# Wikinaut/agrep

Measured on NVIDIA H100. Metric: text_scan_throughput, higher is better.
Workload: dtype u32 bitwise

## Files before the change

### agrep_b200/csrc/refine.cu

```cuda
#include "scan_internal.cuh"


#define REFINE_MAXG  8
int refine_launch_u32a(int nrows, const RefineParams &P, unsigned &grid, cudaStream_t st);
int refine_launch_u32b(int nrows, const RefineParams &P, unsigned &grid, cudaStream_t st);
int refine_launch_u64(int nrows, const RefineParams &P, unsigned &grid, cudaStream_t st);
int refine_launch_costs(bool narrow, int nrows, const RefineParams &P, unsigned &grid, cudaStream_t st);

__global__ void __launch_bounds__(REFINE_THREADS)
k_compact_ranges(const uint32_t *bitmap, uint64_t n_words, const uint64_t *range_offsets, uint64_t *list, uint64_t cap)
{
	const uint32_t lane = threadIdx.x & 31;
	const uint64_t warp = ((uint64_t)blockIdx.x * REFINE_THREADS + threadIdx.x) >> 5, nwarps = ((uint64_t)gridDim.x * REFINE_THREADS) >> 5;
	const uint64_t n_groups = (n_words + 31) / 32, per = (n_groups + nwarps - 1) / nwarps;
	const uint64_t g_begin = warp * per < n_groups ? warp * per : n_groups, g_end = (g_begin + per < n_groups) ? g_begin + per : n_groups;
	uint64_t at = range_offsets[warp];
	for (uint64_t g0 = g_begin; g0 < g_end; g0 += 8) {
		uint32_t wd[8];
#pragma unroll
		for (int u = 0; u < 8; u++) { const uint64_t w = (g0 + u) * 32 + lane; wd[u] = (g0 + u < g_end && w < n_words) ? bitmap[w] : 0u; }
#pragma unroll
		for (int u = 0; u < 8; u++) {
			const uint32_t word = wd[u];
			if (!__ballot_sync(0xffffffffu, word != 0)) continue;
			const uint64_t w = (g0 + u) * 32 + lane;
			uint32_t c = __popc(word), pre = c;
#pragma unroll
			for (int o = 1; o < 32; o <<= 1) { uint32_t v = __shfl_up_sync(0xffffffffu, pre, o); if (lane >= (uint32_t)o) pre += v; }
			const uint32_t total = __shfl_sync(0xffffffffu, pre, 31);
			uint64_t mine = at + (pre - c);
			for (uint32_t b = word; b; b &= b - 1) { if (mine < cap) list[mine] = w * 32 + (uint64_t)(__ffs(b) - 1); mine++; }
			at += total;
		}
	}
}

static bool refine_geometry(const agb_desc &d, RefineParams &P)
{
	if (!front_usable(d) || !d.refine) return false;
	int max_off = 0, min_off = 1 << 30;
	for (int i = 0; i < d.n_anchors; i++) { max_off = std::max(max_off, (int)d.anchor_off[i]); min_off = std::min(min_off, (int)d.anchor_off[i]); }
	for (int i = 0; i < d.n_anchors3; i++) { max_off = std::max(max_off, (int)d.anchor3_off[i]); min_off = std::min(min_off, (int)d.anchor3_off[i]); }
	P.lo_off = max_off + d.k;
	P.hi_off = 15 + d.pat_len - min_off + d.k;
	P.gb = (P.lo_off + 15) / 16;
	P.ng = P.gb + (P.hi_off + 15) / 16;
	if (P.ng < P.gb + 2) P.ng = P.gb + 2;
	const int pw = (d.pat_len + 3) / 4, ngc = (d.engine != AGB_ENGINE_ASEARCH1 && d.M <= 31 && pw <= 4) ? 4 : REFINE_MAXG;
	if (!(P.ng <= ngc && max_off <= 31 && d.pat_len >= 1 && d.pat_len <= 64)) return false;
	const int na = d.n_anchors + d.n_anchors3;
	if (na > 16) return false;
	uint32_t val[16], msk[16]; int off[16];
	for (int i = 0; i < d.n_anchors; i++) { val[i] = d.anchor[i]; msk[i] = d.anchor_mask; off[i] = d.anchor_off[i]; }
	for (int i = 0; i < d.n_anchors3; i++) { val[d.n_anchors + i] = d.anchor3[i]; msk[d.n_anchors + i] = 0x00FFFFFFu; off[d.n_anchors + i] = d.anchor3_off[i]; }
	for (int i = 0; i < na; i++) for (int j = 0; j < i; j++) if ((val[i] & msk[j]) == val[j] || (val[j] & msk[i]) == val[i]) return false;
	uint32_t mul = 0x9E3779B1u;
	for (int attempt = 0; attempt < 4096; attempt++, mul = mul * 0x2C1B3C6Du + 0x297A2D39u) {
		int8_t slot[32]; bool ok = true;
		memset(slot, 0, sizeof slot);
		mul |= 1u;
		for (int i = 0; i < na && ok; i++) {
			const uint32_t h = (val[i] * mul) >> 27;
			if (slot[h]) ok = false; else slot[h] = (int8_t)(i + 1);
		}
		if (!ok) continue;
// ... 5 lines not shown
		return true;
	}
	return false;
}

static void refine_t1_setup(const agb_desc &d, RefineParams &P)
{
	uint8_t lit[64]; bool is_lit[64]; bool fold = false; int n_lit = 0;
	for (int j = 0; j < d.pat_len; j++) {
		const uint64_t bit = 1ull << (d.M - (d.L + 2 + j));
		int cnt = 0, c0 = -1, c1 = -1;
		for (int c = 0; c < 256; c++) if (d.mask[c] & bit) { if (cnt == 0) c0 = c; else if (cnt == 1) c1 = c; cnt++; }
		is_lit[j] = false; lit[j] = 0;
		if (cnt == 1 && c0 < 0x80) { is_lit[j] = true; lit[j] = (uint8_t)c0; }
		else if (cnt == 2 && (c0 ^ c1) == 0x20 && c1 < 0x80) { is_lit[j] = true; lit[j] = (uint8_t)(c0 | 0x20); fold = true; }
		if (is_lit[j]) n_lit++;
	}
	P.t1 = 0;
	if (n_lit <= d.k + 1) return;
	P.t1 = 1; P.t1_fold = fold ? 0x20202020u : 0u;
	for (int w = 0; w < 16; w++) { P.t1_pat[w] = 0; P.t1_care[w] = 0; }
	for (int j = 0; j < d.pat_len; j++) if (is_lit[j]) {
		P.t1_pat[j >> 2] |= (uint32_t)(fold ? (lit[j] | 0x20) : lit[j]) << (8 * (j & 3));
		P.t1_care[j >> 2] |= 0x80u << (8 * (j & 3));
	}
}

int refine_launch(const agb_desc &d, Workspace &W, const void *d_text, uint64_t n, cudaStream_t st, bool *ran)
{
	RefineParams P; memset(&P, 0, sizeof P);
	*ran = false;
	if (n == 0 || !refine_geometry(d, P)) return AGB_OK;
	const uint64_t n_chunks = (n + 15) / 16, n_words = (n_chunks + 31) / 32;
	P.text = (const uint8_t *)d_text; P.bitmap = W.bitmap; P.out = W.bitmap2; P.warp_counts = W.range_counts;
	P.n = n; P.n_chunks = n_chunks; P.n_words = n_words; P.desc = W.d_desc;
	P.fold = d.anchor_fold; P.amask = d.anchor_mask; P.na = d.n_anchors; P.k = d.k; P.pat_len = d.pat_len;
	for (int i = 0; i < d.n_anchors; i++) { P.anchor[i] = d.anchor[i]; P.off[i] = d.anchor_off[i]; }
	{
		bool distinct = true;
		for (int i = 0; i < d.n_anchors; i++) for (int j = 0; j < i; j++) if (d.anchor[i] == d.anchor[j]) distinct = false;
		P.one = 1; P.scale = 1;
		for (int i = d.anchor_len; i < 4; i++) P.scale <<= 8;
		P.poly = (distinct && poly_setup(d.anchor, d.n_anchors, 8 * d.anchor_len, P.coef)) ? 1 : 0;
		P.n3 = 0;
		if (d.n_anchors3) {
			uint32_t c3[AGB_MAXANCHOR];
			if (!P.poly || !poly_setup(d.anchor3, d.n_anchors3, 24, c3)) return AGB_OK;
			P.n3 = d.n_anchors3;
			for (int i = 0; i < d.n_anchors3; i++) P.coef3[i] = c3[i];
		}
	}
	refine_t1_setup(d, P);
	unsigned grid = refine_grid(W, n);
	P.sm_count = W.sm_count;
	const bool costs = d.engine == AGB_ENGINE_ASEARCH1, narrow = d.M <= 31;
	int rc = costs ? refine_launch_costs(narrow, d.nrows, P, grid, st)
	       : !narrow ? refine_launch_u64(d.nrows, P, grid, st)
	       : d.nrows <= 4 ? refine_launch_u32a(d.nrows, P, grid, st) : refine_launch_u32b(d.nrows, P, grid, st);
	if (rc) return AGB_ERR_ARG;
	g_launches++;
	CUDA_TRY(cudaGetLastError());
	W.refine_ctas = grid;
	*ran = true;
	return AGB_OK;
}

unsigned refine_grid(const Workspace &W, uint64_t n)
{
	const uint64_t n_chunks = (n + 15) / 16, n_words = (n_chunks + 31) / 32, groups = (n_words + 31) / 32;
	unsigned grid = (unsigned)std::min<uint64_t>((groups + 3) / 4, (uint64_t)W.sm_count * 16);
	return grid ? grid : 1;
}

int compact_ranges_launch(Workspace &W, uint64_t n, cudaStream_t st)
{
	const uint64_t n_chunks = (n + 15) / 16, n_words = (n_chunks + 31) / 32;
	const unsigned grid = W.refine_ctas;
	k_compact_ranges<<<grid, REFINE_THREADS, 0, st>>>(W.bitmap2, n_words, W.range_offsets, W.cand, W.cand_cap); g_launches++;
	CUDA_TRY(cudaGetLastError());
	return AGB_OK;
}
```

### agrep_b200/csrc/refine_kernel.cuh

```cuda
#ifndef AGB_REFINE_KERNEL_CUH
#define AGB_REFINE_KERNEL_CUH
#include "automaton.cuh"

#define REFINE_RING1 544
#define REFINE_RING2 64
#define REFINE_RING3 128
#define REFINE_MAXG  8
#define REFINE_PAD   32

struct AnchorTable { int8_t idx[32]; uint32_t val[16], mask[16]; int8_t off[16]; int n; };
__device__ __forceinline__ uint32_t hit_windows_tab(const uint32_t (&x)[5], const AnchorTable &A)
{
	uint32_t hits = 0;
#pragma unroll
	for (int w = 0; w < 4; w++) {
		const uint32_t wv[4] = { x[w], __funnelshift_r(x[w], x[w + 1], 8), __funnelshift_r(x[w], x[w + 1], 16), __funnelshift_r(x[w], x[w + 1], 24) };
		for (int a = 0; a < A.n; a++) {
			const uint32_t V = A.val[a], M = A.mask[a];
#pragma unroll
			for (int j = 0; j < 4; j++) if ((wv[j] & M) == V) hits |= 1u << (4 * w + j);
		}
	}
	return hits;
}
// ... 93 lines not shown
		for (int i = 0; i < NWT; i++) W[i] = __funnelshift_r(W[i], W[i + 1], 8);
	}
	int miss = 0;
#pragma unroll
	for (int w = 0; w < NW; w++) miss += __popc(acc[w] & P.t1_care[w]);
	return miss <= P.k;
}

template <typename T, int NR, bool COSTS>
__device__ __forceinline__ bool window_passes(const uint8_t *bytes, const bool run, const int wlen, const T init0,
                                              const T *mask, const DevConsts<T> &C)
{
	T S[NR];
#pragma unroll
	for (int r = 0; r < NR; r++) S[r] = init0;
	int q = 0;
	for (; q + 4 <= wlen; q += 4) {
		int c[4];
#pragma unroll
		for (int i = 0; i < 4; i++) c[i] = run ? (int)__ldg(bytes + q + i) : 0;
		T m[4];
#pragma unroll
		for (int i = 0; i < 4; i++) m[i] = mask[c[i]];
#pragma unroll
		for (int i = 0; i < 4; i++) rows_step<T, NR, COSTS>(S, m[i], C);
	}
	for (; q < wlen; q++) {
		const int c = run ? (int)__ldg(bytes + q) : 0;
		rows_step<T, NR, COSTS>(S, mask[c], C);
	}
	return run && (S[NR - 1] & C.endpos) != 0;
}

struct Refill { uint32_t word, next_word; uint32_t half; };
__device__ __forceinline__ void refine_refill(const RefineParams &P, Refill &R, uint32_t *ring, uint32_t &count, uint32_t lane,
                                              uint64_t &g, uint64_t g_begin, uint64_t g_end)
{
	if (R.half == 0) {
		const uint64_t w = g * 32 + lane;
		R.word = R.next_word;
		if (w < P.n_words) P.out[w] = 0u;
		R.next_word = (g + 1 < g_end && w + 32 < P.n_words) ? P.bitmap[w + 32] : 0u;
	}
	const uint32_t word = ((lane >> 4) == R.half) ? R.word : 0u;
	uint32_t c = __popc(word), pre = c;
#pragma unroll
	for (int o = 1; o < 32; o <<= 1) { uint32_t v = __shfl_up_sync(0xffffffffu, pre, o); if (lane >= (uint32_t)o) pre += v; }
	const uint32_t total = __shfl_sync(0xffffffffu, pre, 31);
	pre += count - c;
	const uint32_t rel0 = (uint32_t)(g - g_begin) * 1024u + lane * 32u;
	for (uint32_t b = word; b; b &= b - 1) ring[pre++] = rel0 + (uint32_t)(__ffs(b) - 1);
	count += total;
	if (R.half) g++;
	R.half ^= 1u;
	__syncwarp();
}

template <typename T, int NR, bool COSTS, int NW>
__global__ void __launch_bounds__(REFINE_THREADS, 6)
k_refine(const RefineParams P)
{
	constexpr int NGC = NW <= 4 ? 4 : REFINE_MAXG;
	constexpr int NWT = NW + (2 * (NR - 1) + 3) / 4;
	extern __shared__ __align__(16) uint32_t s_strip[];
	__shared__ RecShared<T, NR> SH;
	__shared__ uint32_t s_ring1[REFINE_THREADS / 32][REFINE_RING1];
	__shared__ uint32_t s_ring2[REFINE_THREADS / 32][REFINE_RING2];
	__shared__ uint32_t s_ring3[REFINE_THREADS / 32][REFINE_RING3];
	__shared__ AnchorTable s_offs;
	if (threadIdx.x == 0) {
#pragma unroll
		for (int i = 0; i < 32; i++) s_offs.idx[i] = (int8_t)(P.hidx64[i >> 3] >> (8 * (i & 7)));
#pragma unroll
		s_offs.n = P.na + P.n3;
#pragma unroll
		for (int i = 0; i < 16; i++) { s_offs.val[i] = P.hval[i]; s_offs.mask[i] = P.hmask[i]; s_offs.off[i] = (int8_t)(P.hoffs64[i >> 3] >> (8 * (i & 7))); }
	}
	DevConsts<T> C;
	shared_init<T, NR>(SH, C, P.desc, REFINE_THREADS);
	const T init0 = mirror<T>((T)P.desc->init0);
	const int wlen = P.pat_len + 2 * P.k;
	const uint32_t lane = threadIdx.x & 31, wib = threadIdx.x >> 5, lt_mask = (1u << lane) - 1u;
	uint32_t *ring1 = s_ring1[wib], *ring2 = s_ring2[wib], *ring3 = s_ring3[wib];
	const int stride_w = P.ng * 4 + 1;
	uint32_t *strip = s_strip + threadIdx.x * stride_w;
	const uint32_t *cw = strip + P.gb * 4;
	const int so0 = P.gb * 16 - 32 - P.k;

	const uint64_t warp = ((uint64_t)blockIdx.x * REFINE_THREADS + threadIdx.x) >> 5, nwarps = ((uint64_t)gridDim.x * REFINE_THREADS) >> 5;
	const uint64_t n_groups = (P.n_words + 31) / 32, per = (n_groups + nwarps - 1) / nwarps;
	const uint64_t g_begin = warp * per < n_groups ? warp * per : n_groups, g_end = (g_begin + per < n_groups) ? g_begin + per : n_groups;
	const uint64_t chunk0 = g_begin * 1024;
	uint32_t rel_lo, rel_hi;
	{
		const int64_t lo_chunk = ((int64_t)P.lo_off + 15) / 16;
		int64_t hi_chunk = ((int64_t)P.n - P.hi_off - 16) / 16;
		if ((int64_t)P.n - P.hi_off - 16 < 0) hi_chunk = -1;
		if (hi_chunk > (int64_t)P.n_chunks - 3) hi_chunk = (int64_t)P.n_chunks - 3;
		const int64_t a = lo_chunk - (int64_t)chunk0, b = hi_chunk - (int64_t)chunk0;
		rel_lo = a < 0 ? 0u : (a > 0x7fffffff ? 0x7fffffffu : (uint32_t)a);
		rel_hi = b < 0 ? 0u : (b > 0x7fffffff ? 0x7fffffffu : (uint32_t)b);
		if (b < 0) rel_lo = 0x7fffffffu;
	}
	const uint4 *text4 = reinterpret_cast<const uint4 *>(P.text) + chunk0;
	uint32_t kept = 0;
	auto keep_chunk = [&](uint32_t rel) {
		const uint64_t chunk = chunk0 + rel;
		const uint32_t bit = 1u << (chunk & 31);
		const uint32_t old = atomicOr(&P.out[chunk >> 5], bit);
		kept += (old & bit) ? 0u : 1u;
	};

	uint32_t n1 = 0, n2 = 0, n3 = 0;
	uint64_t g = g_begin;
	Refill RF; RF.word = 0; RF.half = 0;
	RF.next_word = (g < g_end && g * 32 + lane < P.n_words) ? P.bitmap[g * 32 + lane] : 0u;
	auto fill1 = [&]() { while (n1 < 32 && g < g_end) refine_refill(P, RF, ring1, n1, lane, g, g_begin, g_end); };
	uint32_t nrel = 0; bool nrun = false, nedge = false; uint4 nx[NGC];
	auto pop_load = [&](uint32_t rel, bool active) {
		nrel = rel;
		nedge = active && (rel < rel_lo || rel > rel_hi);
		nrun = active && !nedge;
		if (nrun) {
			const uint4 *src = text4 + ((int64_t)rel - P.gb);
#pragma unroll
			for (int gi = 0; gi < NGC; gi++) if (gi < P.ng) nx[gi] = __ldg(src + gi);
		}
	};
	auto to_strip = [&]() {
#pragma unroll
		for (int gi = 0; gi < NGC; gi++) if (gi < P.ng) {
			strip[gi * 4 + 0] = nx[gi].x; strip[gi * 4 + 1] = nx[gi].y; strip[gi * 4 + 2] = nx[gi].z; strip[gi * 4 + 3] = nx[gi].w;
		}
	};
	auto count_push = [&](uint32_t rel, uint32_t code, bool run) {
		const bool pass = run && (!P.t1 || band_count_passes<NW, NWT, COSTS ? 0 : 2 * (NR - 1) + 1>(P, strip, so0 + (int)code));
		const uint32_t pm = __ballot_sync(0xffffffffu, pass);
		if (pass) ring3[n3 + __popc(pm & lt_mask)] = (rel << 6) | code;
		n3 += __popc(pm);
	};
	auto walk_batch = [&]() {
		const uint32_t m = n3 < 32 ? n3 : 32;
		const bool run = lane < m;
		const uint32_t e = run ? ring3[n3 - m + lane] : 0u;
		n3 -= m;
		const uint8_t *wbytes = P.text + ((int64_t)(chunk0 + (e >> 6)) * 16 + (int64_t)(e & 63u) - 32 - P.k);
		if (window_passes<T, NR, COSTS>(run ? wbytes : P.text, run, wlen, init0, SH.mask, C)) keep_chunk(e >> 6);
		__syncwarp();
	};
	auto more_batch = [&]() {
		const uint32_t m = n2 < 32 ? n2 : 32;
		const bool run = lane < m;
		const uint32_t e = run ? ring2[n2 - m + lane] : 0u;
		n2 -= m;
		const uint32_t rel = e >> 6, first = e & 63u;
		if (run) {
			const uint4 *src = text4 + ((int64_t)rel - P.gb);
#pragma unroll
			for (int gi = 0; gi < NGC; gi++) if (gi < P.ng) {
				const uint4 v = __ldg(src + gi);
				strip[gi * 4 + 0] = v.x; strip[gi * 4 + 1] = v.y; strip[gi * 4 + 2] = v.z; strip[gi * 4 + 3] = v.w;
			}
		}
		uint32_t hits = 0;
		if (run) {
			const uint32_t x[5] = { cw[0] | P.fold, cw[1] | P.fold, cw[2] | P.fold, cw[3] | P.fold, cw[4] | P.fold };
			hits = P.n3 ? hit_windows_tab(x, s_offs) : hit_windows(x, P);
			hits &= hits - 1;
		}
		uint32_t seen1 = first, seen2 = first;
		for (int it = 0; it < 3; it++) {
			if (!__ballot_sync(0xffffffffu, hits != 0)) break;
			uint32_t code = first; bool fresh = false;
			if (hits) {
				code = start_code(cw, __ffs(hits) - 1, P, s_offs);
				hits &= hits - 1;
				fresh = code != first && code != seen1 && code != seen2;
				seen2 = seen1; seen1 = code;
			}
			count_push(rel, code, fresh);
		}
		if (hits) keep_chunk(rel);
		__syncwarp();
	};
	auto pop1 = [&]() {
		const uint32_t m = n1 < 32 ? n1 : 32;
		const bool active = lane < m;
		pop_load(active ? ring1[n1 - m + lane] : 0u, active);
		n1 -= m;
	};

	bool have = false;
	for (;;) {
		if (n3 >= 32) { walk_batch(); continue; }
		if (n2 >= 32) { more_batch(); continue; }
		if (!have) {
			fill1();
			if (n1 == 0) break;
			pop1(); have = true;
			continue;
		}
		const uint32_t crel = nrel; const bool crun = nrun, cedge = nedge;
		if (crun) to_strip();
		fill1();
		have = n1 != 0;
		if (have) pop1();
		if (cedge) keep_chunk(crel);
		uint32_t hits = 0, code = 0;
		if (crun) {
			const uint32_t x[5] = { cw[0] | P.fold, cw[1] | P.fold, cw[2] | P.fold, cw[3] | P.fold, cw[4] | P.fold };
			hits = P.n3 ? hit_windows_tab(x, s_offs) : hit_windows(x, P);
			if (hits) code = start_code(cw, __ffs(hits) - 1, P, s_offs);
		}
		count_push(crel, code, hits != 0);
		{
			uint32_t rest = hits & (hits - 1);
			if (rest && !(rest & (rest - 1)) && start_code(cw, __ffs(rest) - 1, P, s_offs) == code) rest = 0;
			const bool more = rest != 0;
			const uint32_t mm = __ballot_sync(0xffffffffu, more);
			if (more) ring2[n2 + __popc(mm & lt_mask)] = (crel << 6) | code;
			n2 += __popc(mm);
		}
		__syncwarp();
	}
	while (n2 || n3) { if (n3 >= 32 || !n2) walk_batch(); else more_batch(); }
	const uint32_t total = __reduce_add_sync(0xffffffffu, kept);
	if (lane == 0) P.warp_counts[warp] = total;
}

template <typename T, int NR, bool COSTS, int NW>
static void launch_refine_nw(const RefineParams &P, unsigned &grid, cudaStream_t st)
{
	const size_t smem = ((size_t)REFINE_THREADS * (P.ng * 4 + 1) + REFINE_PAD) * sizeof(uint32_t);
	int per_sm = 0;
	if (cudaOccupancyMaxActiveBlocksPerMultiprocessor(&per_sm, k_refine<T, NR, COSTS, NW>, REFINE_THREADS, smem) != cudaSuccess || per_sm < 1) per_sm = 4;
	grid = std::min<unsigned>(grid, (unsigned)per_sm * (unsigned)P.sm_count);
	if (!grid) grid = 1;
	k_refine<T, NR, COSTS, NW><<<grid, REFINE_THREADS, smem, st>>>(P);
}
template <typename T, int NR, bool COSTS>
static void launch_refine_one(const RefineParams &P, unsigned &grid, cudaStream_t st)
{
	const int pw = (P.pat_len + 3) / 4;
	if (COSTS) { if (sizeof(T) == 4) launch_refine_nw<T, NR, COSTS, 8>(P, grid, st); else launch_refine_nw<T, NR, COSTS, 16>(P, grid, st); return; }
	if (sizeof(T) == 4) {
		if (pw <= 2) launch_refine_nw<T, NR, COSTS, 2>(P, grid, st);
		else if (pw == 3) launch_refine_nw<T, NR, COSTS, 3>(P, grid, st);
		else if (pw == 4) launch_refine_nw<T, NR, COSTS, 4>(P, grid, st);
		else if (pw <= 6) launch_refine_nw<T, NR, COSTS, 6>(P, grid, st);
		else launch_refine_nw<T, NR, COSTS, 8>(P, grid, st);
	} else {
		if (pw <= 8) launch_refine_nw<T, NR, COSTS, 8>(P, grid, st);
		else if (pw <= 12) launch_refine_nw<T, NR, COSTS, 12>(P, grid, st);
// ... 6 lines not shown
```

### agrep_b200/csrc/scan.cu

```cuda
#include "scan_internal.cuh"
#include "corpus.h"
#include <unistd.h>
#include <fcntl.h>
#include <sys/stat.h>
#include <functional>
#include <memory>
#include <mutex>
#include <thread>

thread_local char g_err[512];
std::atomic<uint64_t> g_launches{0};

extern "C" const char *agb_last_error(void) { return g_err; }
extern "C" const char *agb_version(void) { return "agrep-b200 0.1 (sm_90a)"; }
extern "C" uint64_t agb_kernel_launches(void) { return g_launches.load(); }
static void host_release(int dev);
extern "C" void agb_shutdown(void)
{
	int cur = 0; cudaGetDevice(&cur);
	for (int dev = 0; dev < 64; dev++) {
		host_release(dev);
		std::lock_guard<std::mutex> lk(g_ws_mu[dev]);
		Workspace &W = g_ws[dev];
		if (!W.totals && !W.bitmap) continue;
		if (cudaSetDevice(dev) != cudaSuccess) { cudaGetLastError(); continue; }
		cudaDeviceSynchronize();
		cudaFree(W.bitmap); cudaFree(W.bitmap2); cudaFree(W.range_counts); cudaFree(W.range_offsets);
		cudaFree(W.tile_counts); cudaFree(W.tile_offsets); cudaFree(W.cand); cudaFree(W.cand_counts); cudaFree(W.cand_offsets);
		cudaFree(W.cand_first); cudaFree(W.scan_sums); cudaFree(W.scan_offs); cudaFree(W.ord_blocks); cudaFree(W.totals);
		cudaFreeHost(W.h_totals); cudaFree(W.d_desc); cudaFree(W.d_gram); cudaFreeHost(W.h_gram);
		cudaFree(W.d_regex);
		if (W.e0) cudaEventDestroy(W.e0); if (W.e1) cudaEventDestroy(W.e1); if (W.e2) cudaEventDestroy(W.e2);
		W = Workspace();
	}
	cudaSetDevice(cur);
}
extern "C" int agb_device_count(void) { int n = 0; if (cudaGetDeviceCount(&n) != cudaSuccess) return 0; return n; }
extern "C" int agb_set_device(int dev) { CUDA_TRY(cudaSetDevice(dev)); return AGB_OK; }


Workspace g_ws[64];
std::mutex g_ws_mu[64];

static int ws_prepare(Workspace &W, uint64_t n)
{
	if (!W.totals) {
		CUDA_TRY(cudaMalloc(&W.totals, 24 * sizeof(unsigned long long)));
		CUDA_TRY(cudaMallocHost(&W.h_totals, 24 * sizeof(unsigned long long)));
		CUDA_TRY(cudaMalloc(&W.d_desc, sizeof(agb_desc)));
		CUDA_TRY(cudaMalloc(&W.range_counts, REFINE_MAX_RANGES * sizeof(uint32_t)));
		CUDA_TRY(cudaMalloc(&W.range_offsets, REFINE_MAX_RANGES * sizeof(uint64_t)));
		CUDA_TRY(cudaEventCreate(&W.e0)); CUDA_TRY(cudaEventCreate(&W.e1)); CUDA_TRY(cudaEventCreate(&W.e2));
		int dev = 0; CUDA_TRY(cudaGetDevice(&dev));
		CUDA_TRY(cudaDeviceGetAttribute(&W.sm_count, cudaDevAttrMultiProcessorCount, dev));
	}
	uint64_t n_chunks = (n + 15) / 16, n_words = (n_chunks + 31) / 32, tiles = (n + std::min<uint64_t>(DENSE_TILE, SL_TILE) - 1) / std::min<uint64_t>(DENSE_TILE, SL_TILE) + 1;
	size_t bb = (size_t)(n_words + FRONT_WORDS_PER_STAGE) * 4;
	if (bb > W.bitmap_bytes) {
		if (W.bitmap) cudaFree(W.bitmap);
		if (W.bitmap2) cudaFree(W.bitmap2);
		W.bitmap = nullptr; W.bitmap2 = nullptr; W.bitmap_bytes = 0;
		CUDA_TRY(cudaMalloc(&W.bitmap, bb));
		CUDA_TRY(cudaMalloc(&W.bitmap2, bb)); W.bitmap_bytes = bb;
	}
	if (tiles + 1 > W.tiles) {
		if (W.tile_counts) cudaFree(W.tile_counts);
		if (W.tile_offsets) cudaFree(W.tile_offsets);
		W.tile_counts = nullptr; W.tile_offsets = nullptr; W.tiles = 0;
		CUDA_TRY(cudaMalloc(&W.tile_counts, (tiles + 1) * sizeof(uint32_t)));
		CUDA_TRY(cudaMalloc(&W.tile_offsets, (tiles + 1) * sizeof(uint64_t)));
		W.tiles = tiles + 1;
	}
	return AGB_OK;
}

static int ws_cand_reserve(Workspace &W, size_t want_cand)
{
	want_cand = std::max<size_t>(want_cand, (size_t)1 << 20);
	if (want_cand > W.cand_cap) {
		want_cand += want_cand / 4;
		if (W.cand) cudaFree(W.cand);
		if (W.cand_counts) cudaFree(W.cand_counts);
		if (W.cand_offsets) cudaFree(W.cand_offsets);
		if (W.cand_first) cudaFree(W.cand_first);
		if (W.scan_sums) cudaFree(W.scan_sums);
		if (W.scan_offs) cudaFree(W.scan_offs);
		W.cand = nullptr; W.cand_counts = nullptr; W.cand_offsets = nullptr; W.cand_first = nullptr; W.cand_cap = 0;
		W.scan_sums = nullptr; W.scan_offs = nullptr; W.scan_cap = 0;
		CUDA_TRY(cudaMalloc(&W.cand_first, want_cand * sizeof(agb_record)));
		W.scan_cap = want_cand / SCAN_BLOCK + 2;
		CUDA_TRY(cudaMalloc(&W.scan_sums, W.scan_cap * sizeof(uint32_t)));
		CUDA_TRY(cudaMalloc(&W.scan_offs, W.scan_cap * sizeof(uint64_t)));
		CUDA_TRY(cudaMalloc(&W.cand, want_cand * sizeof(uint64_t)));
		CUDA_TRY(cudaMalloc(&W.cand_counts, want_cand * sizeof(uint32_t)));
		CUDA_TRY(cudaMalloc(&W.cand_offsets, want_cand * sizeof(uint64_t)));
		W.cand_cap = want_cand;
// ... 22 lines not shown
		CUDA_TRY(cudaMemcpyAsync(W.d_regex, tab, bytes, cudaMemcpyHostToDevice, st));
		CUDA_TRY(cudaStreamSynchronize(st));
		memcpy(W.h_regex, tab, bytes); W.regex_bytes = bytes;
	}
	W.regex_tail = rx->tail;
	return AGB_OK;
}

static int list_stage(const agb_desc &d, Workspace &W, RecParams &P, bool want_list, cudaStream_t st)
{
	P.cand = W.cand; P.cand_cap = W.cand_cap; P.tile_counts = W.cand_counts; P.tile_offsets = W.cand_offsets;
	P.cand_first = want_list ? W.cand_first : nullptr;
	const unsigned grid = (unsigned)std::min<uint64_t>((W.cand_cap + REC_THREADS - 1) / REC_THREADS, (uint64_t)W.sm_count * 16);
	if (launch_records_list(d, P, grid, st)) return AGB_ERR_ARG;
	CUDA_TRY(cudaGetLastError());
	if (want_list) {
		const unsigned nb = (unsigned)((W.cand_cap + SCAN_BLOCK - 1) / SCAN_BLOCK);
		k_scan_partial<<<nb, 1024, 0, st>>>(W.cand_counts, W.cand_cap, W.scan_sums, W.totals + 12);
		k_scan_tiles<<<1, 1024, 0, st>>>(W.scan_sums, W.scan_offs, nb, nullptr);
		k_scan_apply<<<nb, 1024, 0, st>>>(W.cand_counts, W.cand_cap, W.scan_offs, W.cand_offsets, W.totals + 12);
		g_launches += 3;
		P.emit = 1;
		if (launch_records_list(d, P, grid, st)) return AGB_ERR_ARG;
		CUDA_TRY(cudaGetLastError());
	}
	return AGB_OK;
}

static int records_launch(const agb_desc &d, Workspace &W, const void *d_text, uint64_t n, bool use_front, bool refined, int want,
                          int want_level, agb_record *d_records, uint64_t capacity, cudaStream_t st, const ShardInfo *sh)
{
	const uint64_t n_chunks = (n + 15) / 16, n_words = (n_chunks + 31) / 32, tiles = (n_words + REC_THREADS - 1) / REC_THREADS;
	RecParams P; memset(&P, 0, sizeof P);
	P.text = (const uint8_t *)d_text; P.bitmap = use_front ? (refined ? W.bitmap2 : W.bitmap) : nullptr;
	P.n = n; P.n_chunks = n_chunks; P.n_words = n_words; P.desc = W.d_desc;
	P.records = d_records; P.capacity = capacity;
	P.totals = W.totals; P.emit = 0; P.levels = (want & AGB_WANT_LEVELS) ? 1 : 0; P.want_level = want_level;
	P.own_lo = sh ? sh->own_lo : INT64_MIN; P.own_hi = sh ? sh->own_hi : INT64_MAX; P.shard_last = sh ? sh->last : 1;
	P.rx_tab = W.d_regex; P.rx_tail = W.regex_tail;
	if (!tiles) return AGB_OK;
	const bool want_list = (want & AGB_WANT_RECORDS) && capacity;
	if (d.engine == AGB_ENGINE_REGEX) {
		P.tile_counts = W.tile_counts; P.tile_offsets = W.tile_offsets;
		const uint64_t rtiles = (n + DENSE_TILE - 1) / DENSE_TILE;
		if (launch_regex(d, P, (unsigned)rtiles, st)) return AGB_ERR_ARG;
		CUDA_TRY(cudaGetLastError());
		if (want_list) {
			k_scan_tiles<<<1, 1024, 0, st>>>(W.tile_counts, W.tile_offsets, rtiles, nullptr); g_launches++;
			P.emit = 1;
			if (launch_regex(d, P, (unsigned)rtiles, st)) return AGB_ERR_ARG;
			CUDA_TRY(cudaGetLastError());
		}
		return AGB_OK;
	}
	if (use_front && refined) {
		int rc = ws_cand_reserve(W, std::max<size_t>(W.cand_hint + W.cand_hint / 4, (size_t)(n_chunks / 512) + 65536)); if (rc) return rc;
		const unsigned ranges = W.refine_ctas * (REFINE_THREADS / 32);
		k_scan_tiles<<<1, 1024, 0, st>>>(W.range_counts, W.range_offsets, ranges, W.totals + 12); g_launches++;
		rc = compact_ranges_launch(W, n, st); if (rc) return rc;
		return list_stage(d, W, P, want_list, st);
	}
	if (use_front) {
		const uint64_t blocks = (n_words + COMPACT_THREADS * COMPACT_WPT - 1) / (COMPACT_THREADS * COMPACT_WPT);
		k_compact_count<<<(unsigned)blocks, COMPACT_THREADS, 0, st>>>(W.bitmap, n_words, W.tile_counts, W.totals); g_launches++;
		k_scan_tiles<<<1, 1024, 0, st>>>(W.tile_counts, W.tile_offsets, blocks, W.totals + 12); g_launches++;
		CUDA_TRY(cudaMemcpyAsync(W.h_totals + 12, W.totals + 12, sizeof(unsigned long long), cudaMemcpyDeviceToHost, st));
		CUDA_TRY(cudaStreamSynchronize(st));
// ... 844 lines not shown
```

### agrep_b200/csrc/scan_internal.cuh

```cuda
#ifndef AGB_SCAN_INTERNAL_CUH
#define AGB_SCAN_INTERNAL_CUH
#include "agrep_b200.h"
#include "pattern_internal.h"
#include <cuda_runtime.h>
#include <stdint.h>
#include <stdio.h>
#include <string.h>
#include <stdlib.h>
#include <atomic>
#include <algorithm>

extern thread_local char g_err[512];
extern std::atomic<uint64_t> g_launches;

#define CUDA_TRY(x) do { cudaError_t e_ = (x); if (e_ != cudaSuccess) { \
	snprintf(g_err, sizeof g_err, "%s failed: %s (%s:%d)", #x, cudaGetErrorString(e_), __FILE__, __LINE__); \
	return AGB_ERR_CUDA; } } while (0)

#define FRONT_THREADS 256
#define FRONT_CH      4
#define FRONT_STAGE_CHUNKS (FRONT_THREADS * FRONT_CH)
#define FRONT_STAGE_BYTES  (FRONT_STAGE_CHUNKS * 16)
#define FRONT_SLOT_BYTES   (FRONT_STAGE_BYTES + 16)
#define FRONT_NST     2
#define FRONT_CTAS_PER_SM 6
#define FRONT_WORDS_PER_STAGE (FRONT_STAGE_CHUNKS / 32)

struct FrontParams {
	const uint8_t *text;
	uint32_t    *bitmap;
	uint64_t     n;
	uint64_t     n_chunks;
	uint64_t     readable;
	uint64_t     stage_begin, stage_end;
	uint32_t     fold, amask;
	uint32_t     one, scale;
	uint32_t     anchor[AGB_MAXANCHOR];
	uint32_t     coef[AGB_MAXANCHOR];
	int          n3;
	uint32_t     s256;
	int          alen;
	uint32_t     coef3[4];
	uint16_t    *nl_blocks;
	uint32_t     delim4, dfold4;
};
#define FRONT_SMEM (FRONT_NST * FRONT_SLOT_BYTES)

#define REFINE_THREADS 128
struct RefineParams {
	const uint8_t *text; const uint32_t *bitmap; uint32_t *out; uint32_t *warp_counts;
	uint64_t n, n_chunks, n_words;
	const agb_desc *desc;
	uint32_t fold, amask; int na, k, pat_len;
	int gb, ng;
	int lo_off, hi_off;
	uint32_t anchor[AGB_MAXANCHOR]; int32_t off[AGB_MAXANCHOR];
	uint32_t coef[AGB_MAXANCHOR]; uint32_t one, scale; int poly;
	int t1, t1_words;
	uint32_t t1_fold, t1_pat[16], t1_care[16];
	uint32_t hmul; uint64_t hidx64[4];
	uint32_t hval[16], hmask[16]; uint64_t hoffs64[2];
	int n3; uint32_t coef3[4];
	int sm_count;
};

#define REC_THREADS 128

struct RecParams {
	const uint8_t  *text;
	const uint32_t *bitmap;
	uint64_t n, n_chunks, n_words;
	const agb_desc *desc;
	uint32_t *tile_counts;
	const uint64_t *tile_offsets;
	agb_record *records; uint64_t capacity;
	unsigned long long *totals;
	const uint64_t *cand; uint64_t cand_cap;
	agb_record *cand_first;
	int emit;
	int levels;
	int want_level;
	int warm;
	int64_t own_lo, own_hi; int shard_last;
// ... 10 lines not shown
#define SL_TILE    (SL_THREADS * SL_PER)
#define SL_APRON   128
#define SL_STRIDE  (SL_PER + 4)
#define SL_SMEM    ((SL_THREADS + 1) * SL_STRIDE + 12)
#define COMPACT_THREADS 256
#define COMPACT_WPT 4
#define SCAN_BLOCK 16384

#define ORD_THREADS 256
#define ORD_TILE    32768
#define ORD_PER     (ORD_TILE / ORD_THREADS)
#define ORD_BLOCK   512

struct OrdParams {
	const uint8_t *text; uint64_t n;
	uint16_t *blocks; uint32_t *tiles; const uint64_t *tile_off;
	agb_record *records; const unsigned long long *totals; uint64_t capacity;
	uint8_t delim[AGB_MAXDELIM + 2], dfold[AGB_MAXDELIM + 2]; int L, kind;
	long long j0;
};

__device__ __forceinline__ bool rec_owned(const RecParams &P, int64_t begin, int L, int64_t close_pos)
{
	const int64_t oe = begin + L - 1;
	if (oe < P.own_lo || oe >= P.own_hi) return false;
	if (!P.shard_last && close_pos >= (int64_t)P.n) P.totals[11] = 1ull;
	return true;
}

#define H2D_SLICE   (64ull << 20)
#define STAGE_BUFS  3
struct Workspace {
	uint32_t *bitmap = nullptr; size_t bitmap_bytes = 0;
	uint32_t *bitmap2 = nullptr;
	uint32_t *range_counts = nullptr; uint64_t *range_offsets = nullptr;
	unsigned refine_ctas = 0;
	uint32_t *d_gram = nullptr; unsigned int *h_gram = nullptr;
	uint64_t plan_key = 0; bool plan_valid = false; agb_desc plan_desc;
	size_t cand_hint = 0;
	uint32_t *tile_counts = nullptr; uint64_t *tile_offsets = nullptr; size_t tiles = 0;
	uint64_t *cand = nullptr; uint32_t *cand_counts = nullptr; uint64_t *cand_offsets = nullptr; agb_record *cand_first = nullptr; size_t cand_cap = 0;
	uint32_t *scan_sums = nullptr; uint64_t *scan_offs = nullptr; size_t scan_cap = 0;
	uint16_t *ord_blocks = nullptr; size_t ord_blocks_cap = 0;
	long long ord_j0 = 0;
	int ord_virt = 0;
	unsigned long long *totals = nullptr;
	unsigned long long *h_totals = nullptr;
	agb_desc *d_desc = nullptr; agb_desc h_desc_copy; bool desc_valid = false;
	cudaEvent_t e0 = nullptr, e1 = nullptr, e2 = nullptr;
	int sm_count = 0;
	uint64_t *d_regex = nullptr; uint64_t h_regex[8 * 256]; size_t regex_bytes = 0; int regex_tail = 0;
};

#include <mutex>
extern Workspace g_ws[64];
extern std::mutex g_ws_mu[64];
int  scan_device_impl(const agb_desc &d, const void *d_text, uint64_t n, int want, int want_level,
                      agb_record *d_records, uint64_t capacity, cudaStream_t st, agb_result *res, const ShardInfo *sh = nullptr,
                      const agb_regex *rx = nullptr);
enum { HALO_SHORT_RIGHT = 1, HALO_SHORT_LEFT = 2 };
int  shard_window_scan(const agb_desc &d, const agb_regex *rx, const void *d_win, uint64_t n_local, uint64_t halo_left, uint64_t halo_right,
                       bool first, bool open_end, bool reaches_end, int want, agb_record *d_records, uint64_t capacity,
                       cudaStream_t st, agb_result *lres, agb_shard_part *part);
int  shard_window_rebase(agb_record *d_records, uint64_t n, long long byte_add, long long ord_add, bool ordinals, cudaStream_t st);
bool front_usable(const agb_desc &d);
bool exact_count_usable(const agb_desc &d);
int  exact_count_launch(const agb_desc &d, Workspace &W, const void *d_text, uint64_t n, cudaStream_t st);
bool poly_setup(const uint32_t *a, int na, int bits, uint32_t *coef);
int  front_launch(const agb_desc &d, Workspace &W, const void *d_text, uint64_t n, uint64_t word_begin, uint64_t word_end, bool slack16, cudaStream_t st, bool count_delims = false);
int  refine_launch(const agb_desc &d, Workspace &W, const void *d_text, uint64_t n, cudaStream_t st, bool *ran);
unsigned refine_grid(const Workspace &W, uint64_t n);
int  compact_ranges_launch(Workspace &W, uint64_t n, cudaStream_t st);
#define REFINE_MAX_RANGES 16384
int  launch_records(const agb_desc &d, const RecParams &P, unsigned grid, cudaStream_t st);
int  launch_dense(const agb_desc &d, const RecParams &P, unsigned grid, cudaStream_t st);
int  launch_records_list(const agb_desc &d, const RecParams &P, unsigned grid, cudaStream_t st);
int  launch_slices(const agb_desc &d, const RecParams &P, unsigned grid, cudaStream_t st);
bool slices_usable(const agb_desc &d);
int  launch_regex(const agb_desc &d, const RecParams &P, unsigned grid, cudaStream_t st);
size_t regex_tables(const agb_desc &d, const agb_regex &rx, uint64_t *out);
__global__ void k_gram_sample(const uint8_t *text, uint64_t n_chunks, uint32_t nblk, uint32_t blk_chunks,
                              int ngram, const uint32_t *gram, const uint32_t *gmask, uint32_t fold, unsigned int *counts,
                              int pair_first, int n_pair);
__global__ void k_compact_count(const uint32_t *bitmap, uint64_t n_words, uint32_t *block_counts, unsigned long long *totals);
__global__ void k_compact_write(const uint32_t *bitmap, uint64_t n_words, const uint64_t *block_offsets, uint64_t *cand, uint64_t cand_cap);
__global__ void k_scan_tiles(const uint32_t *counts, uint64_t *offsets, uint64_t n_tiles, unsigned long long *total);
__global__ void k_scan_partial(const uint32_t *counts, uint64_t n, uint32_t *block_sums, const unsigned long long *n_dev);
__global__ void k_scan_apply(const uint32_t *counts, uint64_t n, const uint64_t *block_offsets, uint64_t *offsets, const unsigned long long *n_dev);
int  front_is_dense(Workspace &W, uint64_t n, cudaStream_t st, bool *dense);
int  ordinals_launch(const agb_desc &d, Workspace &W, const void *d_text, uint64_t n, agb_record *d_records, uint64_t capacity, cudaStream_t st, bool blocks_counted = false);
int  ordinals_reserve(const agb_desc &d, Workspace &W, uint64_t n);
#endif
```

Baseline: 2300.

## Replace refine bitmap scanning with per-stage compact candidate lists and survivor masks

Adds a pre-pass kernel that turns each 1024-chunk stage of the candidate bitmap into a short uint16 list (up to 56 entries) with a count. The refine kernel then fills its work ring directly from these lists, and records survivors in a per-stage 64-bit mask instead of a second full bitmap. Dense stages fall back to the bitmap, with an overflow flag. This removes the second bitmap, its zeroing, and the bitmap scan in refill and compaction, at the cost of an extra launch, 64-bit ring entries in shared memory, and more complex logic.

```diff
diff --git a/agrep_b200/csrc/refine.cu b/agrep_b200/csrc/refine.cu
--- a/agrep_b200/csrc/refine.cu
+++ b/agrep_b200/csrc/refine.cu
@@ -8,29 +8,67 @@
 int refine_launch_costs(bool narrow, int nrows, const RefineParams &P, unsigned &grid, cudaStream_t st);
 
 __global__ void __launch_bounds__(REFINE_THREADS)
-k_compact_ranges(const uint32_t *bitmap, uint64_t n_words, const uint64_t *range_offsets, uint64_t *list, uint64_t cap)
+k_compact_ranges(const unsigned long long *surv, const uint16_t *lists, const uint32_t *bitmap, uint64_t n_words,
+                 const uint64_t *range_offsets, uint64_t *list, uint64_t cap)
 {
 	const uint32_t lane = threadIdx.x & 31;
 	const uint64_t warp = ((uint64_t)blockIdx.x * REFINE_THREADS + threadIdx.x) >> 5, nwarps = ((uint64_t)gridDim.x * REFINE_THREADS) >> 5;
 	const uint64_t n_groups = (n_words + 31) / 32, per = (n_groups + nwarps - 1) / nwarps;
 	const uint64_t g_begin = warp * per < n_groups ? warp * per : n_groups, g_end = (g_begin + per < n_groups) ? g_begin + per : n_groups;
 	uint64_t at = range_offsets[warp];
-	for (uint64_t g0 = g_begin; g0 < g_end; g0 += 8) {
-		uint32_t wd[8];
+	for (uint64_t b = g_begin; b < g_end; b += 32) {
+		const uint64_t s = b + lane;
+		const unsigned long long m = s < g_end ? surv[s] : 0ull;
+		if (!__ballot_sync(0xffffffffu, m != 0)) continue;
+		const uint32_t ovf = __ballot_sync(0xffffffffu, (m & SURV_OVERFLOW) != 0);
+		uint32_t c = (uint32_t)__popcll(m & ~SURV_OVERFLOW);
+		for (uint32_t o = ovf; o; o &= o - 1) {
+			const uint32_t l = __ffs(o) - 1;
+			const uint64_t w = (b + l) * 32 + lane;
+			const uint32_t t = __reduce_add_sync(0xffffffffu, (uint32_t)__popc(w < n_words ? bitmap[w] : 0u));
+			if (lane == l) c = t;
+		}
+		uint32_t pre = c;
 #pragma unroll
-		for (int u = 0; u < 8; u++) { const uint64_t w = (g0 + u) * 32 + lane; wd[u] = (g0 + u < g_end && w < n_words) ? bitmap[w] : 0u; }
+		for (int o = 1; o < 32; o <<= 1) { uint32_t v = __shfl_up_sync(0xffffffffu, pre, o); if (lane >= (uint32_t)o) pre += v; }
+		const uint32_t total = __shfl_sync(0xffffffffu, pre, 31);
+		uint64_t mine = at + (pre - c);
+		if (m && !(m & SURV_OVERFLOW)) {
+			const uint16_t *e = lists + s * FLAG_LIST_MAX;
+			for (unsigned long long r = m; r; r &= r - 1) { if (mine < cap) list[mine] = s * 1024 + e[__ffsll((long long)r) - 1]; mine++; }
+		}
+		for (uint32_t o = ovf; o; o &= o - 1) {
+			const uint32_t l = __ffs(o) - 1;
+			uint64_t pos = __shfl_sync(0xffffffffu, mine, l);
+			const uint64_t w = (b + l) * 32 + lane;
+			const uint32_t word = w < n_words ? bitmap[w] : 0u;
+			uint32_t cw = __popc(word), pw = cw;
 #pragma unroll
-		for (int u = 0; u < 8; u++) {
-			const uint32_t word = wd[u];
-			if (!__ballot_sync(0xffffffffu, word != 0)) continue;
-			const uint64_t w = (g0 + u) * 32 + lane;
-			uint32_t c = __popc(word), pre = c;
+			for (int k = 1; k < 32; k <<= 1) { uint32_t v = __shfl_up_sync(0xffffffffu, pw, k); if (lane >= (uint32_t)k) pw += v; }
+			pos += pw - cw;
+			for (uint32_t r = word; r; r &= r - 1) { if (pos < cap) list[pos] = w * 32 + (uint64_t)(__ffs(r) - 1); pos++; }
+		}
+		at += total;
+	}
+}
+
+__global__ void __launch_bounds__(256)
+k_flag_lists(const uint32_t *bitmap, uint64_t n_words, uint16_t *counts, uint16_t *lists)
+{
+	const uint32_t lane = threadIdx.x & 31;
+	const uint64_t n_stages = (n_words + 31) / 32, nwarps = ((uint64_t)gridDim.x * blockDim.x) >> 5;
+	for (uint64_t sg = ((uint64_t)blockIdx.x * blockDim.x + threadIdx.x) >> 5; sg < n_stages; sg += nwarps) {
+		const uint64_t wi = sg * 32 + lane;
+		const uint32_t w = wi < n_words ? bitmap[wi] : 0u;
+		const uint32_t c = __popc(w);
+		uint32_t pre = c;
 #pragma unroll
-			for (int o = 1; o < 32; o <<= 1) { uint32_t v = __shfl_up_sync(0xffffffffu, pre, o); if (lane >= (uint32_t)o) pre += v; }
-			const uint32_t total = __shfl_sync(0xffffffffu, pre, 31);
-			uint64_t mine = at + (pre - c);
-			for (uint32_t b = word; b; b &= b - 1) { if (mine < cap) list[mine] = w * 32 + (uint64_t)(__ffs(b) - 1); mine++; }
-			at += total;
+		for (int o = 1; o < 32; o <<= 1) { const uint32_t v = __shfl_up_sync(0xffffffffu, pre, o); if (lane >= (uint32_t)o) pre += v; }
+		const uint32_t total = __shfl_sync(0xffffffffu, pre, 31);
+		if (lane == 0) counts[sg] = (uint16_t)total;
+		if (total <= FLAG_LIST_MAX) {
+			uint16_t *out = lists + sg * FLAG_LIST_MAX + (pre - c);
+			for (uint32_t b = w; b; b &= b - 1) *out++ = (uint16_t)(lane * 32 + __ffs(b) - 1);
 		}
 	}
 }
@@ -102,7 +140,8 @@
 	*ran = false;
 	if (n == 0 || !refine_geometry(d, P)) return AGB_OK;
 	const uint64_t n_chunks = (n + 15) / 16, n_words = (n_chunks + 31) / 32;
-	P.text = (const uint8_t *)d_text; P.bitmap = W.bitmap; P.out = W.bitmap2; P.warp_counts = W.range_counts;
+	P.text = (const uint8_t *)d_text; P.bitmap = W.bitmap; P.warp_counts = W.range_counts;
+	P.flag_counts = W.flag_counts; P.flag_lists = W.flag_lists; P.surv = W.surv;
 	P.n = n; P.n_chunks = n_chunks; P.n_words = n_words; P.desc = W.d_desc;
 	P.fold = d.anchor_fold; P.amask = d.anchor_mask; P.na = d.n_anchors; P.k = d.k; P.pat_len = d.pat_len;
 	for (int i = 0; i < d.n_anchors; i++) { P.anchor[i] = d.anchor[i]; P.off[i] = d.anchor_off[i]; }
@@ -121,6 +160,12 @@
 		}
 	}
 	refine_t1_setup(d, P);
+	{
+		const uint64_t n_stages = (n_words + 31) / 32;
+		const unsigned lg = (unsigned)std::min<uint64_t>((n_stages + 7) / 8, (uint64_t)W.sm_count * 16);
+		k_flag_lists<<<lg ? lg : 1, 256, 0, st>>>(W.bitmap, n_words, W.flag_counts, W.flag_lists); g_launches++;
+		CUDA_TRY(cudaGetLastError());
+	}
 	unsigned grid = refine_grid(W, n);
 	P.sm_count = W.sm_count;
 	const bool costs = d.engine == AGB_ENGINE_ASEARCH1, narrow = d.M <= 31;
@@ -146,7 +191,7 @@
 {
 	const uint64_t n_chunks = (n + 15) / 16, n_words = (n_chunks + 31) / 32;
 	const unsigned grid = W.refine_ctas;
-	k_compact_ranges<<<grid, REFINE_THREADS, 0, st>>>(W.bitmap2, n_words, W.range_offsets, W.cand, W.cand_cap); g_launches++;
+	k_compact_ranges<<<grid, REFINE_THREADS, 0, st>>>(W.surv, W.flag_lists, W.bitmap, n_words, W.range_offsets, W.cand, W.cand_cap); g_launches++;
 	CUDA_TRY(cudaGetLastError());
 	return AGB_OK;
 }
diff --git a/agrep_b200/csrc/refine_kernel.cuh b/agrep_b200/csrc/refine_kernel.cuh
--- a/agrep_b200/csrc/refine_kernel.cuh
+++ b/agrep_b200/csrc/refine_kernel.cuh
@@ -149,27 +149,70 @@
 	return run && (S[NR - 1] & C.endpos) != 0;
 }
 
-struct Refill { uint32_t word, next_word; uint32_t half; };
+#define REFINE_REL_MASK ((1u << 26) - 1u)
+#define REFINE_J_BITMAP 63u
+
+__device__ __forceinline__ uint32_t list_entry(const uint4 v, int h)
+{
+	const uint32_t w = h < 2 ? v.x : h < 4 ? v.y : h < 6 ? v.z : v.w;
+	return (h & 1) ? w >> 16 : w & 0xFFFFu;
+}
+
+struct Refill { uint32_t cnt, next_cnt; uint64_t blk; uint32_t word, half; };
+__device__ __forceinline__ uint32_t refill_count(const RefineParams &P, uint64_t s, uint64_t g_end)
+{
+	if (s >= g_end) return 0u;
+	P.surv[s] = 0ull;
+	return P.flag_counts[s];
+}
 __device__ __forceinline__ void refine_refill(const RefineParams &P, Refill &R, uint32_t *ring, uint32_t &count, uint32_t lane,
                                               uint64_t &g, uint64_t g_begin, uint64_t g_end)
 {
-	if (R.half == 0) {
-		const uint64_t w = g * 32 + lane;
-		R.word = R.next_word;
-		if (w < P.n_words) P.out[w] = 0u;
-		R.next_word = (g + 1 < g_end && w + 32 < P.n_words) ? P.bitmap[w + 32] : 0u;
-	}
-	const uint32_t word = ((lane >> 4) == R.half) ? R.word : 0u;
-	uint32_t c = __popc(word), pre = c;
-#pragma unroll
-	for (int o = 1; o < 32; o <<= 1) { uint32_t v = __shfl_up_sync(0xffffffffu, pre, o); if (lane >= (uint32_t)o) pre += v; }
-	const uint32_t total = __shfl_sync(0xffffffffu, pre, 31);
-	pre += count - c;
-	const uint32_t rel0 = (uint32_t)(g - g_begin) * 1024u + lane * 32u;
-	for (uint32_t b = word; b; b &= b - 1) ring[pre++] = rel0 + (uint32_t)(__ffs(b) - 1);
-	count += total;
-	if (R.half) g++;
-	R.half ^= 1u;
+	if (g == R.blk + 32) { R.blk += 32; R.cnt = R.next_cnt; R.next_cnt = refill_count(P, R.blk + 32 + lane, g_end); }
+	const uint32_t p = (uint32_t)(g - R.blk);
+	const uint32_t rel_stage = (uint32_t)(g - g_begin) * 1024u;
+	if (__shfl_sync(0xffffffffu, R.cnt, p) > FLAG_LIST_MAX) {
+		if (R.half == 0) {
+			const uint64_t w = g * 32 + lane;
+			R.word = w < P.n_words ? P.bitmap[w] : 0u;
+			if (w < P.n_words) P.bitmap[w] = 0u;
+		}
+		const uint32_t word = ((lane >> 4) == R.half) ? R.word : 0u;
+		uint32_t c = __popc(word), pre = c;
+#pragma unroll
+		for (int o = 1; o < 32; o <<= 1) { uint32_t v = __shfl_up_sync(0xffffffffu, pre, o); if (lane >= (uint32_t)o) pre += v; }
+		const uint32_t total = __shfl_sync(0xffffffffu, pre, 31);
+		pre += count - c;
+		const uint32_t rel0 = rel_stage + lane * 32u;
+		for (uint32_t b = word; b; b &= b - 1) ring[pre++] = (rel0 + (uint32_t)(__ffs(b) - 1)) | (REFINE_J_BITMAP << 26);
+		count += total;
+		if (R.half) g++;
+		R.half ^= 1u;
+	} else {
+		const bool mine = lane >= p;
+		const uint32_t stop = __ballot_sync(0xffffffffu, mine && (R.cnt > FLAG_LIST_MAX || R.blk + lane >= g_end));
+		const uint32_t q = stop ? (uint32_t)__ffs(stop) - 1u : 32u;
+		const uint32_t v = (mine && lane < q) ? R.cnt : 0u;
+		uint32_t incl = v;
+#pragma unroll
+		for (int o = 1; o < 32; o <<= 1) { uint32_t t = __shfl_up_sync(0xffffffffu, incl, o); if (lane >= (uint32_t)o) incl += t; }
+		const bool take = mine && lane < q && incl <= (uint32_t)REFINE_RING1 - count;
+		const uint32_t taken = __popc(__ballot_sync(0xffffffffu, take));
+		const uint32_t total = __shfl_sync(0xffffffffu, incl, p + taken - 1);
+		if (take && v) {
+			const uint4 *src = reinterpret_cast<const uint4 *>(P.flag_lists + (R.blk + lane) * FLAG_LIST_MAX);
+			uint32_t *dst = ring + count + incl - v;
+			const uint32_t rel0 = rel_stage + (lane - p) * 1024u;
+#pragma unroll 1
+			for (uint32_t j = 0; j < v; j += 8) {
+				const uint4 e = __ldg(src + j / 8);
+#pragma unroll
+				for (int h = 0; h < 8; h++) if (j + h < v) dst[j + h] = (rel0 + list_entry(e, h)) | ((j + h) << 26);
+			}
+		}
+		count += total;
+		g += taken;
+	}
 	__syncwarp();
 }
 
@@ -182,8 +225,8 @@
 	extern __shared__ __align__(16) uint32_t s_strip[];
 	__shared__ RecShared<T, NR> SH;
 	__shared__ uint32_t s_ring1[REFINE_THREADS / 32][REFINE_RING1];
-	__shared__ uint32_t s_ring2[REFINE_THREADS / 32][REFINE_RING2];
-	__shared__ uint32_t s_ring3[REFINE_THREADS / 32][REFINE_RING3];
+	__shared__ uint64_t s_ring2[REFINE_THREADS / 32][REFINE_RING2];
+	__shared__ uint64_t s_ring3[REFINE_THREADS / 32][REFINE_RING3];
 	__shared__ AnchorTable s_offs;
 	if (threadIdx.x == 0) {
 #pragma unroll
@@ -198,7 +241,8 @@
 	const T init0 = mirror<T>((T)P.desc->init0);
 	const int wlen = P.pat_len + 2 * P.k;
 	const uint32_t lane = threadIdx.x & 31, wib = threadIdx.x >> 5, lt_mask = (1u << lane) - 1u;
-	uint32_t *ring1 = s_ring1[wib], *ring2 = s_ring2[wib], *ring3 = s_ring3[wib];
+	uint32_t *ring1 = s_ring1[wib];
+	uint64_t *ring2 = s_ring2[wib], *ring3 = s_ring3[wib];
 	const int stride_w = P.ng * 4 + 1;
 	uint32_t *strip = s_strip + threadIdx.x * stride_w;
 	const uint32_t *cw = strip + P.gb * 4;
@@ -221,21 +265,29 @@
 	}
 	const uint4 *text4 = reinterpret_cast<const uint4 *>(P.text) + chunk0;
 	uint32_t kept = 0;
-	auto keep_chunk = [&](uint32_t rel) {
-		const uint64_t chunk = chunk0 + rel;
-		const uint32_t bit = 1u << (chunk & 31);
-		const uint32_t old = atomicOr(&P.out[chunk >> 5], bit);
-		kept += (old & bit) ? 0u : 1u;
+	auto keep_chunk = [&](uint32_t cid) {
+		const uint64_t chunk = chunk0 + (cid & REFINE_REL_MASK);
+		const uint32_t j = cid >> 26;
+		if (j == REFINE_J_BITMAP) {
+			const uint32_t bit = 1u << (chunk & 31);
+			const uint32_t old = atomicOr(&P.bitmap[chunk >> 5], bit);
+			if (!(old & bit)) { kept++; atomicOr(&P.surv[chunk >> 10], SURV_OVERFLOW); }
+		} else {
+			const unsigned long long bit = 1ull << j;
+			const unsigned long long old = atomicOr(&P.surv[chunk >> 10], bit);
+			kept += (old & bit) ? 0u : 1u;
+		}
 	};
 
 	uint32_t n1 = 0, n2 = 0, n3 = 0;
 	uint64_t g = g_begin;
-	Refill RF; RF.word = 0; RF.half = 0;
-	RF.next_word = (g < g_end && g * 32 + lane < P.n_words) ? P.bitmap[g * 32 + lane] : 0u;
+	Refill RF; RF.word = 0; RF.half = 0; RF.blk = g_begin;
+	RF.cnt = refill_count(P, g_begin + lane, g_end); RF.next_cnt = refill_count(P, g_begin + 32 + lane, g_end);
 	auto fill1 = [&]() { while (n1 < 32 && g < g_end) refine_refill(P, RF, ring1, n1, lane, g, g_begin, g_end); };
 	uint32_t nrel = 0; bool nrun = false, nedge = false; uint4 nx[NGC];
-	auto pop_load = [&](uint32_t rel, bool active) {
-		nrel = rel;
+	auto pop_load = [&](uint32_t cid, bool active) {
+		nrel = cid;
+		const uint32_t rel = cid & REFINE_REL_MASK;
 		nedge = active && (rel < rel_lo || rel > rel_hi);
 		nrun = active && !nedge;
 		if (nrun) {
@@ -250,29 +302,30 @@
 			strip[gi * 4 + 0] = nx[gi].x; strip[gi * 4 + 1] = nx[gi].y; strip[gi * 4 + 2] = nx[gi].z; strip[gi * 4 + 3] = nx[gi].w;
 		}
 	};
-	auto count_push = [&](uint32_t rel, uint32_t code, bool run) {
+	auto count_push = [&](uint32_t cid, uint32_t code, bool run) {
 		const bool pass = run && (!P.t1 || band_count_passes<NW, NWT, COSTS ? 0 : 2 * (NR - 1) + 1>(P, strip, so0 + (int)code));
 		const uint32_t pm = __ballot_sync(0xffffffffu, pass);
-		if (pass) ring3[n3 + __popc(pm & lt_mask)] = (rel << 6) | code;
+		if (pass) ring3[n3 + __popc(pm & lt_mask)] = ((uint64_t)cid << 6) | code;
 		n3 += __popc(pm);
 	};
 	auto walk_batch = [&]() {
 		const uint32_t m = n3 < 32 ? n3 : 32;
 		const bool run = lane < m;
-		const uint32_t e = run ? ring3[n3 - m + lane] : 0u;
+		const uint64_t e = run ? ring3[n3 - m + lane] : 0ull;
 		n3 -= m;
-		const uint8_t *wbytes = P.text + ((int64_t)(chunk0 + (e >> 6)) * 16 + (int64_t)(e & 63u) - 32 - P.k);
-		if (window_passes<T, NR, COSTS>(run ? wbytes : P.text, run, wlen, init0, SH.mask, C)) keep_chunk(e >> 6);
+		const uint32_t cid = (uint32_t)(e >> 6);
+		const uint8_t *wbytes = P.text + ((int64_t)(chunk0 + (cid & REFINE_REL_MASK)) * 16 + (int64_t)(e & 63u) - 32 - P.k);
+		if (window_passes<T, NR, COSTS>(run ? wbytes : P.text, run, wlen, init0, SH.mask, C)) keep_chunk(cid);
 		__syncwarp();
 	};
 	auto more_batch = [&]() {
 		const uint32_t m = n2 < 32 ? n2 : 32;
 		const bool run = lane < m;
-		const uint32_t e = run ? ring2[n2 - m + lane] : 0u;
+		const uint64_t e = run ? ring2[n2 - m + lane] : 0ull;
 		n2 -= m;
-		const uint32_t rel = e >> 6, first = e & 63u;
+		const uint32_t cid = (uint32_t)(e >> 6), first = (uint32_t)e & 63u;
 		if (run) {
-			const uint4 *src = text4 + ((int64_t)rel - P.gb);
+			const uint4 *src = text4 + ((int64_t)(cid & REFINE_REL_MASK) - P.gb);
 #pragma unroll
 			for (int gi = 0; gi < NGC; gi++) if (gi < P.ng) {
 				const uint4 v = __ldg(src + gi);
@@ -295,9 +348,9 @@
 				fresh = code != first && code != seen1 && code != seen2;
 				seen2 = seen1; seen1 = code;
 			}
-			count_push(rel, code, fresh);
-		}
-		if (hits) keep_chunk(rel);
+			count_push(cid, code, fresh);
+		}
+		if (hits) keep_chunk(cid);
 		__syncwarp();
 	};
 	auto pop1 = [&]() {
@@ -335,7 +388,7 @@
 			if (rest && !(rest & (rest - 1)) && start_code(cw, __ffs(rest) - 1, P, s_offs) == code) rest = 0;
 			const bool more = rest != 0;
 			const uint32_t mm = __ballot_sync(0xffffffffu, more);
-			if (more) ring2[n2 + __popc(mm & lt_mask)] = (crel << 6) | code;
+			if (more) ring2[n2 + __popc(mm & lt_mask)] = ((uint64_t)crel << 6) | code;
 			n2 += __popc(mm);
 		}
 		__syncwarp();
diff --git a/agrep_b200/csrc/scan.cu b/agrep_b200/csrc/scan.cu
--- a/agrep_b200/csrc/scan.cu
+++ b/agrep_b200/csrc/scan.cu
@@ -25,7 +25,7 @@
 		if (!W.totals && !W.bitmap) continue;
 		if (cudaSetDevice(dev) != cudaSuccess) { cudaGetLastError(); continue; }
 		cudaDeviceSynchronize();
-		cudaFree(W.bitmap); cudaFree(W.bitmap2); cudaFree(W.range_counts); cudaFree(W.range_offsets);
+		cudaFree(W.bitmap); cudaFree(W.flag_counts); cudaFree(W.flag_lists); cudaFree(W.surv); cudaFree(W.range_counts); cudaFree(W.range_offsets);
 		cudaFree(W.tile_counts); cudaFree(W.tile_offsets); cudaFree(W.cand); cudaFree(W.cand_counts); cudaFree(W.cand_offsets);
 		cudaFree(W.cand_first); cudaFree(W.scan_sums); cudaFree(W.scan_offs); cudaFree(W.ord_blocks); cudaFree(W.totals);
 		cudaFreeHost(W.h_totals); cudaFree(W.d_desc); cudaFree(W.d_gram); cudaFreeHost(W.h_gram);
@@ -57,11 +57,13 @@
 	uint64_t n_chunks = (n + 15) / 16, n_words = (n_chunks + 31) / 32, tiles = (n + std::min<uint64_t>(DENSE_TILE, SL_TILE) - 1) / std::min<uint64_t>(DENSE_TILE, SL_TILE) + 1;
 	size_t bb = (size_t)(n_words + FRONT_WORDS_PER_STAGE) * 4;
 	if (bb > W.bitmap_bytes) {
-		if (W.bitmap) cudaFree(W.bitmap);
-		if (W.bitmap2) cudaFree(W.bitmap2);
-		W.bitmap = nullptr; W.bitmap2 = nullptr; W.bitmap_bytes = 0;
+		cudaFree(W.bitmap); cudaFree(W.flag_counts); cudaFree(W.flag_lists); cudaFree(W.surv);
+		W.bitmap = nullptr; W.flag_counts = nullptr; W.flag_lists = nullptr; W.surv = nullptr; W.bitmap_bytes = 0;
+		const size_t stages = bb / (FRONT_WORDS_PER_STAGE * 4);
 		CUDA_TRY(cudaMalloc(&W.bitmap, bb));
-		CUDA_TRY(cudaMalloc(&W.bitmap2, bb)); W.bitmap_bytes = bb;
+		CUDA_TRY(cudaMalloc(&W.flag_counts, stages * sizeof(uint16_t)));
+		CUDA_TRY(cudaMalloc(&W.flag_lists, stages * FLAG_LIST_MAX * sizeof(uint16_t)));
+		CUDA_TRY(cudaMalloc(&W.surv, stages * sizeof(unsigned long long))); W.bitmap_bytes = bb;
 	}
 	if (tiles + 1 > W.tiles) {
 		if (W.tile_counts) cudaFree(W.tile_counts);
@@ -150,7 +152,7 @@
 {
 	const uint64_t n_chunks = (n + 15) / 16, n_words = (n_chunks + 31) / 32, tiles = (n_words + REC_THREADS - 1) / REC_THREADS;
 	RecParams P; memset(&P, 0, sizeof P);
-	P.text = (const uint8_t *)d_text; P.bitmap = use_front ? (refined ? W.bitmap2 : W.bitmap) : nullptr;
+	P.text = (const uint8_t *)d_text; P.bitmap = use_front && !refined ? W.bitmap : nullptr;
 	P.n = n; P.n_chunks = n_chunks; P.n_words = n_words; P.desc = W.d_desc;
 	P.records = d_records; P.capacity = capacity;
 	P.totals = W.totals; P.emit = 0; P.levels = (want & AGB_WANT_LEVELS) ? 1 : 0; P.want_level = want_level;
diff --git a/agrep_b200/csrc/scan_internal.cuh b/agrep_b200/csrc/scan_internal.cuh
--- a/agrep_b200/csrc/scan_internal.cuh
+++ b/agrep_b200/csrc/scan_internal.cuh
@@ -44,11 +44,14 @@
 	uint16_t    *nl_blocks;
 	uint32_t     delim4, dfold4;
 };
+#define FLAG_LIST_MAX 56
 #define FRONT_SMEM (FRONT_NST * FRONT_SLOT_BYTES)
 
 #define REFINE_THREADS 128
 struct RefineParams {
-	const uint8_t *text; const uint32_t *bitmap; uint32_t *out; uint32_t *warp_counts;
+	const uint8_t *text; uint32_t *bitmap; uint32_t *warp_counts;
+	const uint16_t *flag_counts, *flag_lists;
+	unsigned long long *surv;
 	uint64_t n, n_chunks, n_words;
 	const agb_desc *desc;
 	uint32_t fold, amask; int na, k, pat_len;
@@ -125,7 +128,8 @@
 #define STAGE_BUFS  3
 struct Workspace {
 	uint32_t *bitmap = nullptr; size_t bitmap_bytes = 0;
-	uint32_t *bitmap2 = nullptr;
+	uint16_t *flag_counts = nullptr, *flag_lists = nullptr;
+	unsigned long long *surv = nullptr;
 	uint32_t *range_counts = nullptr; uint64_t *range_offsets = nullptr;
 	unsigned refine_ctas = 0;
 	uint32_t *d_gram = nullptr; unsigned int *h_gram = nullptr;
@@ -164,6 +168,7 @@
 int  refine_launch(const agb_desc &d, Workspace &W, const void *d_text, uint64_t n, cudaStream_t st, bool *ran);
 unsigned refine_grid(const Workspace &W, uint64_t n);
 int  compact_ranges_launch(Workspace &W, uint64_t n, cudaStream_t st);
+#define SURV_OVERFLOW (1ull << 63)
 #define REFINE_MAX_RANGES 16384
 int  launch_records(const agb_desc &d, const RecParams &P, unsigned grid, cudaStream_t st);
 int  launch_dense(const agb_desc &d, const RecParams &P, unsigned grid, cudaStream_t st);
```

Result: no change. 2317, median of 6 (+0.7%).
